# NVIDIA/flowtron

Hardware: AMD Instinct MI355X
Metric: mel-frames/sec training (2-flow, 80-mel) (higher is better)
Workload: dtype bf16; 1 GPU; BASELINE configs[1]: 2-flow LJS config.json model, per-GPU batch 32, T_max=862, L_max=157, attn-prior + CTC on, fwd+loss+bwd+clip+RAdam; global_batch=32, parallelism=dp1, mfma_operands=bf16, storage=fp32, skipped_steps=0

## Files before the change

### flowtron_amd/_lib.py

```python
from __future__ import annotations

import ctypes as C
import os

import torch

_HERE = os.path.dirname(os.path.abspath(__file__))
LIB_PATH = os.path.join(_HERE, "libflowtron_hip.so")

FT_F32, FT_BF16, FT_F16 = 0, 1, 2
GEMM_SPLITK = 1
GEMM_SPLITK_DET = 2
GEMM_C16 = 4
ACT_NONE, ACT_TANH, ACT_RELU, ACT_SIGMOID = 0, 1, 2, 3

_p, _i, _l, _f, _sz, _d = C.c_void_p, C.c_int, C.c_int64, C.c_float, C.c_size_t, C.c_double


class GemmArgs(C.Structure):
    _fields_ = [("A", _p), ("B", _p), ("C", _p), ("bias", _p),
                ("M", _i), ("N", _i), ("K", _i), ("batch", _i),
                ("sAm", _l), ("sAk", _l), ("sBk", _l), ("sBn", _l), ("ldc", _l),
                ("bsA", _l), ("bsB", _l), ("bsC", _l),
                ("alpha", _f), ("beta", _f), ("act", _i), ("mode", _i), ("flags", _i),
# ... 9 lines not shown


class GemmImgPlan(C.Structure):
    _fields_ = [(n, _i) for n in ("tile_rows", "stage_k", "gather", "atomics", "det", "splits", "chunk_w")]


class GemmImgGroupPlan(C.Structure):
    _fields_ = [(n, _i) for n in ("tile_rows", "splits", "ksteps", "atomics", "launch", "unit0", "tiles")]


GEMM_GROUP_MAX = 48


class LstmFwdRole(C.Structure):
    _fields_ = [("gx", _p), ("lens", _p), ("y", _p), ("ldy", _l), ("gates", _p), ("cell", _p), ("wimg", _p), ("state_h", _p), ("state_c", _p),
                ("B", C.c_int32), ("ldb", C.c_int32), ("t0", C.c_int32), ("t1", C.c_int32), ("gx16", C.c_int32)]


class LstmBwdRole(C.Structure):
    _fields_ = [("dy", _p), ("ldy", _l), ("lens", _p), ("gates", _p), ("cell", _p), ("dgx", _p), ("wimg", _p),
                ("dimg", _p), ("dimg_ld", _l), ("dimg_rows", _l), ("dbias", _p), ("state_da", _p), ("state_dc", _p),
                ("B", C.c_int32), ("ldb", C.c_int32), ("t0", C.c_int32), ("t1", C.c_int32), ("carry_in", C.c_int32)]


class ImgDesc(C.Structure):
    _fields_ = [("src", _p), ("ld", _l), ("rows", _l), ("cols", _l), ("dst", _p), ("kind", _i)]


class CummAttnArgs(C.Structure):
    _fields_ = [(n, _p) for n in ("text", "Q", "V", "w_key", "v", "w1", "b1", "w2", "b2", "in_lens", "ctx", "attn", "logprob",
                                  "cumm_all", "kproj_all", "work")] + [("work_bytes", _sz)] + [
        (n, _i) for n in ("T", "B", "L", "E", "A", "NF", "K1", "K2")] + [("temperature", _f), ("mode", _i), ("persist_status", _p)]


class DecodeArgs(C.Structure):
    _fields_ = [(n, _p) for n in (
        "att_w_ih", "att_w_hh", "att_b_ih", "att_b_hh", "w_query", "v", "K", "V",
# ... 60 lines not shown
    "ft_lstm_persist_workspace_bytes": ([_i, _i], _sz),
    "ft_lstm_persist_debug_prof": ([_p], _i),
    "ft_lstm_persist_bwd": ([_p, _l, _p, _p, _p, _p, _p, _p, _p, _i, _i, _i, _i, _p], _i),
    "ft_bilstm_persist_supported": ([_i, _i], _i),
    "ft_bilstm_persist_workspace_bytes": ([_i, _i], C.c_size_t),
    "ft_bilstm_persist_debug_prof": ([_p], _i),
    "ft_bilstm_persist_fwd": ([_p, _p, _p, _p, _p, _p, _l, _p, _p, _p, _p, _p, _p, _i, _i, _i, _p], _i),
    "ft_bilstm_persist_bwd": ([_p, _l, _p, _p, _p, _p, _p, _p, _p, _p, _p, _p, _p, _i, _i, _i, _p], _i),
    "ft_lstm_persist_bwd_img": ([_p, _l, _p, _p, _p, _p, _p, _p, _p, _i, _i, _i, _i, _p, _l, _l, _p, _p], _i),
    "ft_lstm_roles_ctx_bytes": ([], _sz),
    "ft_lstm_roles_wimg_bytes": ([_i], _sz),
    "ft_lstm_roles_ctx_init": ([_p, _p], _i),
    "ft_lstm_roles_debug_prof": ([_p], _i),
    "ft_lstm_roles_prepare_fwd": ([_p, _p, _i, _p], _i),
    "ft_lstm_roles_prepare_bwd": ([_p, _p, _i, _p], _i),
    "ft_lstm_roles_fwd": ([C.POINTER(LstmFwdRole), _i, _i, _i, _p, _i, _p, _i, _p], _i),
    "ft_lstm_roles_bwd": ([C.POINTER(LstmBwdRole), _i, _i, _i, _p, _i, _p, _i, _p], _i),
    "ft_lstm2_supported": ([_i, _i], _i),
    "ft_lstm2_workspace_bytes": ([_i, _i], _sz),
    "ft_lstm2_seq_fwd": ([_p] * 13 + [_i, _i, _i, _p], _i),
    "ft_lstm2_seq_bwd": ([_p] * 12 + [_i, _i, _i, _p], _i),
    "ft_lstm_bidir_supported": ([_i, _i], _i),
    "ft_lstm_bidir_seq_fwd": ([_p] * 6 + [_l] + [_p] * 6 + [_i, _i, _i, _p], _i),
    "ft_lstm_bidir_seq_bwd": ([_p, _l] + [_p] * 11 + [_i, _i, _i, _p], _i),
    "ft_cumm_attn_workspace_bytes": ([_i] * 10, _sz),
    "ft_cumm_attn_fused": ([C.POINTER(CummAttnArgs)], _i),
    "ft_cumm_attn_debug_prof": ([_p], _i),
    "ft_cumm_attn_fwd": ([C.POINTER(CummAttnArgs), _p], _i),
    "ft_cumm_attn_bwd": ([C.POINTER(CummAttnArgs)] + [_p] * 13, _i),
    "ft_attention_fwd": ([_p] * 8 + [_i, _i, _i, _i, _f, _p], _i),
# ... 72 lines not shown
    "ft_radam_step": ([_p, _p, _p, _p, _l, _p, _d, _d, _d, _d, _d, _d, _d, _i, _p, _p], _i),
    "ft_radam_step_dev": ([_p, _p, _p, _p, _l, _p, _d, _d, _d, _d, _d, _d, _i, _p, _p], _i),
    "ft_poison_if_nonzero": ([_p, _p, _p], _i),
    "ft_mixture_nll_work_floats": ([_i, _i, _i, _i], _sz),
    "ft_mixture_nll_fwd": ([_p] * 5 + [_i, _l] + [_p] * 4 + [_i] * 5 + [_p], _i),
    "ft_mixture_nll_bwd": ([_p] * 13 + [_i] * 5 + [_p], _i),
    "ft_time_pool_fwd": ([_p, _p, _p, _i, _i, _i, _p], _i),
    "ft_time_pool_bwd": ([_p, _p, _p, _i, _i, _i, _p], _i),
    "ft_softmax_rows_fwd": ([_p, _p, _i, _i, _p], _i),
    "ft_softmax_rows_bwd": ([_p, _p, _p, _i, _i, _p], _i),
    "ft_mixture_sample": ([_p] * 6 + [_i] * 5 + [_f, _p], _i),
}
MIXTURE_MAX_C = 64

OP16_TWINS = ("ft_gemm", "ft_bf16_image", "ft_bf16_image_colsum", "ft_bf16_image_colsum_acc", "ft_bf16_image_rows_acc", "ft_bf16_image_rows_act_bwd_acc", "ft_gemm_img", "ft_gemm_img_group", "ft_bf16_image_rows", "ft_bf16_image_rows_into", "ft_bf16_image_rows_act_bwd", "ft_img_gemv_rows", "ft_img_gemv_rows_bwd", "ft_lstm_seq_fwd", "ft_lstm_seq_bwd",
              "ft_lstm_persist_bwd", "ft_lstm_persist_bwd_img", "ft_lstm_roles_prepare_fwd", "ft_lstm_roles_prepare_bwd", "ft_lstm_roles_fwd", "ft_lstm_roles_bwd", "ft_lstm2_seq_fwd", "ft_lstm2_seq_bwd",
              "ft_lstm_bidir_seq_fwd", "ft_lstm_bidir_seq_bwd", "ft_bilstm_persist_fwd", "ft_bilstm_persist_bwd")
for _n in OP16_TWINS:
    SIGNATURES[_n + "_f16"] = SIGNATURES[_n]

_lib = None


def lib():
    global _lib
    if _lib is None:
        if not os.path.exists(LIB_PATH):
            raise RuntimeError(
                "libflowtron_hip.so is missing (%s). Build it with `python -m flowtron_amd.build` "
                "(hipcc --offload-arch=gfx950). There is no CPU/PyTorch fallback." % LIB_PATH)
        l = C.CDLL(LIB_PATH)
# ... 60 lines not shown
```

### flowtron_amd/csrc/lstm_roles.hip

```cpp
#include "lstm_persist_common.h"

namespace {

constexpr int CPG = 32, UPC = 32, TPC = 8;
constexpr int RMAX = 16;
constexpr int SBMAX = 32;
constexpr int RRING = 8, RDIST = 6;

constexpr int NBUF = 4;
constexpr size_t FWD_SET_DW = (size_t)8 * NBUF * (NCHUNK * 32 * RMAX / 2);
constexpr size_t BWD_SET_FL = (size_t)2 * 8 * 32 * 32 * 32 * RMAX;
constexpr size_t CTX_BYTES = 256 + 2 * FWD_SET_DW * 4 + 2 * BWD_SET_FL * 4;

struct FwdRoleP {
    const float* gx; const int* lens; float* y; long ldy; float* gates; float* cell;
    const unsigned short* wfrag;
    float* st_h; float* st_c;
    int B, LB, t0, t1;
};
struct FwdLaunchP {
    FwdRoleP role[2];
    int nroles;
    unsigned* hand;
    unsigned* census;
    int phase, reset_rows;
    int* status; long timeout_ticks; long* prof;
};

template <typename T>
__device__ __forceinline__ T* uniform_ptr(T* p) {
    const unsigned long long v = (unsigned long long)p;
    const unsigned lo = (unsigned)__builtin_amdgcn_readfirstlane((int)(unsigned)v), hi = (unsigned)__builtin_amdgcn_readfirstlane((int)(unsigned)(v >> 32));
    return (T*)(((unsigned long long)hi << 32) | lo);
}

__device__ __forceinline__ void dma16(const float* src, unsigned lds_addr) {
    unsigned keep;
    asm volatile("s_mov_b32 %0, m0\n\ts_mov_b32 m0, %2\n\ts_nop 0\n\tglobal_load_lds_dwordx4 %1, off\n\ts_mov_b32 m0, %0"
                 : "=&s"(keep) : "v"(src), "s"((unsigned)__builtin_amdgcn_readfirstlane((int)lds_addr)) : "memory");
}

__device__ __forceinline__ void preset_other(uint4* other, size_t n16, unsigned* census_other, int wg, int tid) {
    const uint4 v = {SENT, SENT, SENT, SENT};
    for (size_t i = (size_t)wg * 256 + tid; i < n16; i += (size_t)NCU * 256) other[i] = v;
    if (wg == 0 && tid < 8) census_other[tid] = 0u;
}

template <int R, bool PROF, bool GX16>
__global__ __launch_bounds__(256, 1) void lstm_roles_fwd_k(FwdLaunchP P) {
    constexpr bool SPLIT = R >= 8;
    constexpr int ERW = SPLIT ? 8 : 4;
    constexpr int EPT = R / ERW;
    constexpr int ETH = SPLIT ? 256 : 128;
    constexpr int NE = R * UPC;
    constexpr int CPL = 16 / R, NLG = 8 / CPL;
    constexpr int SBF = R == 16 ? 4 : SBMAX * 4 / R;
    constexpr int SB = GX16 ? 2 * SBF : SBF;
    constexpr int DWG = NCHUNK * 32 * R / 2;
    extern __shared__ __attribute__((aligned(16))) float smem[];
    float (*red)[4][TPC][R][20] = reinterpret_cast<float (*)[4][TPC][R][20]>(smem);
    float* gxs = smem + 2 * 4 * TPC * R * 20;
    float* outs = gxs + SBF * 4 * NE;

    const int tid = threadIdx.x, lane = tid & 63, wave = tid >> 6;
// ... 28 lines not shown
#pragma unroll
    for (int e = 0; e < EPT; ++e) {
        const int eb = b0 + er0 + ERW * e;
        ev[e] = erole && eb < B;
        len[e] = ev[e] ? p.lens[eb] : 0;
    }
    int tg = 0;
    for (int r = 0; r < R; ++r) {
        const int bb = b0 + r;
        if (bb < B) { const int l = p.lens[bb]; tg = l > tg ? l : tg; }
    }
    tg = tg < t1 ? tg : t1;
    tg = __builtin_amdgcn_readfirstlane(tg);

    const int wu = __builtin_amdgcn_readfirstlane(wave);
    auto burst = [&](int t) {
        __syncthreads();
        const int nst = (tg - t) < SB ? (tg - t) : SB;
        const unsigned dst0 = (unsigned)(size_t)(lds_void*)gxs;
        if constexpr (GX16) {
            const unsigned short* gx16 = reinterpret_cast<const unsigned short*>(p.gx);
#pragma unroll
            for (int kk = 0; kk < SB * R / 16; ++kk) {
                const int c = 4 * kk + wu, st = c / (R / 4), pi = c % (R / 4);
                const int f = pi * 512 + lane * 8, gate = f / NE, row = (f % NE) >> 5, unit = f & 31;
                if (st < nst && b0 + row < B)
                    dma16(reinterpret_cast<const float*>(gx16 + (((size_t)(t + st) * LB + b0 + row) * 4 + gate) * PH + q * UPC + unit),
                          dst0 + (unsigned)(st * 4 * NE * 2 + pi * 1024));
            }
        } else {
#pragma unroll
            for (int kk = 0; kk < SB * R / 8; ++kk) {
                const int c = 4 * kk + wu, st = c / (R / 2), pi = c % (R / 2);
                const int f = pi * 256 + lane * 4, gate = f / NE, row = (f % NE) >> 5, unit = f & 31;
                if (st < nst && b0 + row < B)
// ... 651 lines not shown
            }
        }
        if (t0 == 0) {
            int Rr = 0;
            for (int bb = 0; bb < B; ++bb) Rr += p.lens[bb] + 1;
            int Rz = (Rr + 32 + 255) & ~255;
            Rz = Rz < p.dimg_rows ? Rz : p.dimg_rows;
            for (int r = Rr + lgrp * CPG + q; r < Rz; r += gpr * CPG) {
                uint4* row = reinterpret_cast<uint4*>(p.dimg + (size_t)r * p.dimg_ld);
                for (int c = tid; c < 4 * PH / 8; c += 256) row[c] = make_uint4(0u, 0u, 0u, 0u);
            }
        }
    }
}

}

#if FT_OPFMT == 0
long* ftint_roles_prof = nullptr;
extern "C" int ft_lstm_roles_debug_prof(void* dev_buf) { ftint_roles_prof = reinterpret_cast<long*>(dev_buf); return FT_OK; }
extern "C" size_t ft_lstm_roles_ctx_bytes(void) { return CTX_BYTES; }
extern "C" size_t ft_lstm_roles_wimg_bytes(int H) { return (size_t)4 * H * H * 2; }
extern "C" int ft_lstm_roles_ctx_init(void* ctx, void* stream) {
    FT_CHECK_ARG(ctx && reinterpret_cast<uintptr_t>(ctx) % 256 == 0);
    hipStream_t st = reinterpret_cast<hipStream_t>(stream);
    FT_CHECK_HIP(hipMemsetAsync(ctx, 0, 256, st));
    FT_CHECK_HIP(hipMemsetAsync(reinterpret_cast<char*>(ctx) + 256, 0xFF, CTX_BYTES - 256, st));
    return FT_OK;
}
#else
// ... 5 lines not shown
extern "C" int FT_OPNAME(ft_lstm_roles_prepare_fwd)(const float* w_hh, void* wimg, int H, void* stream) {
    FT_CHECK_ARG(w_hh && wimg && H == PH && reinterpret_cast<uintptr_t>(wimg) % 256 == 0);
    hipLaunchKernelGGL(make_wfrag_fwd_ug, dim3(2048), dim3(256), 0, reinterpret_cast<hipStream_t>(stream), w_hh,
                       reinterpret_cast<unsigned short*>(wimg), H, WfragAux{nullptr, 0ul, 0u, nullptr});
    FT_CHECK_LAUNCH();
    return FT_OK;
}
extern "C" int FT_OPNAME(ft_lstm_roles_prepare_bwd)(const float* w_hh, void* wimg, int H, void* stream) {
    FT_CHECK_ARG(w_hh && wimg && H == PH && reinterpret_cast<uintptr_t>(wimg) % 256 == 0);
    hipLaunchKernelGGL(make_wfrag_rs, dim3(2048), dim3(256), 0, reinterpret_cast<hipStream_t>(stream), w_hh,
                       reinterpret_cast<unsigned short*>(wimg), H, WfragAux{nullptr, 0ul, 0u, nullptr});
    FT_CHECK_LAUNCH();
    return FT_OK;
}

template <typename K, typename PT>
static int roles_launch(K kern, size_t lds, const PT& P, hipStream_t st) {
    FT_CHECK_HIP(hipFuncSetAttribute(reinterpret_cast<const void*>(kern), hipFuncAttributeMaxDynamicSharedMemorySize, (int)lds));
    hipLaunchKernelGGL(kern, dim3(NCU), dim3(256), lds, st, P);
    return FT_OK;
}

extern "C" int FT_OPNAME(ft_lstm_roles_fwd)(const ft_lstm_fwd_role* roles, int n_roles, int rows_per_group, int reset_rows, void* ctx, int phase,
                                            int32_t* status, int H, void* stream) {
    FT_CHECK_ARG(roles && ctx && status && (n_roles == 1 || n_roles == 2) && reinterpret_cast<uintptr_t>(ctx) % 256 == 0 && phase >= 0);
    const int R = rows_per_group;
    FT_CHECK_ARG((R == 4 || R == 8 || R == 16) && (reset_rows == 4 || reset_rows == 8 || reset_rows == 16) && reset_rows >= 4);
    if (H != PH || !ft_lstm_persist_supported(8, H))
        return ft_fail(FT_EUNSUPPORTED, "ft_lstm_roles_fwd: needs H == 1024 and a 256-CU device (H=%d)", H);
    FwdLaunchP P{};
    bool any = false, g16 = false;
    for (int i = 0; i < n_roles; ++i) {
        const ft_lstm_fwd_role& r = roles[i];
        FT_CHECK_ARG(r.gx && r.lens && r.y && r.wimg && r.B >= 1 && r.B <= (8 / n_roles) * R && r.ldb >= r.B && r.ldy >= H);
        FT_CHECK_ARG((r.gates == nullptr) == (r.cell == nullptr) && (r.state_h == nullptr) == (r.state_c == nullptr));
        FT_CHECK_ARG(r.t0 >= 0 && r.t1 >= r.t0 && (r.t0 == 0 || r.state_h) && reinterpret_cast<uintptr_t>(r.gx) % 16 == 0);
        P.role[i] = FwdRoleP{reinterpret_cast<const float*>(r.gx), r.lens, r.y, (long)r.ldy, r.gates, r.cell, reinterpret_cast<const unsigned short*>(r.wimg),
                             r.state_h, r.state_c, r.B, r.ldb, r.t0, r.t1};
        FT_CHECK_ARG(i == 0 || (r.gx16 != 0) == g16);
        g16 = r.gx16 != 0;
        any = any || r.t1 > r.t0;
    }
    if (!any) return ft_fail(FT_EINVAL, "ft_lstm_roles_fwd: every window is empty (t1 == t0): nothing to launch");
    char* base = reinterpret_cast<char*>(ctx);
    P.nroles = n_roles;
    P.census = reinterpret_cast<unsigned*>(base);
    P.hand = reinterpret_cast<unsigned*>(base + 256);
    P.phase = phase; P.reset_rows = reset_rows;
    P.status = status; P.timeout_ticks = 100000000L / 2; P.prof = ftint_roles_prof;
    hipStream_t st = reinterpret_cast<hipStream_t>(stream);
    auto lds = [](int R_, int SB_) { return sizeof(float) * ((size_t)2 * 4 * TPC * R_ * 20 + (size_t)SB_ * 4 * R_ * UPC + (size_t)2 * 6 * R_ * UPC); };
    int rc;
    const bool pf = ftint_roles_prof != nullptr;
#define FT_ROLES_FWD(R_, SB_) \
    (g16 ? (pf ? roles_launch(lstm_roles_fwd_k<R_, true, true>, lds(R_, SB_), P, st) : roles_launch(lstm_roles_fwd_k<R_, false, true>, lds(R_, SB_), P, st)) \
         : (pf ? roles_launch(lstm_roles_fwd_k<R_, true, false>, lds(R_, SB_), P, st) : roles_launch(lstm_roles_fwd_k<R_, false, false>, lds(R_, SB_), P, st)))
    if (R == 4) rc = FT_ROLES_FWD(4, 32);
    else if (R == 8) rc = FT_ROLES_FWD(8, 16);
    else rc = FT_ROLES_FWD(16, 4);
#undef FT_ROLES_FWD
    if (rc != FT_OK) return rc;
    FT_CHECK_LAUNCH();
    return FT_OK;
}

extern "C" int FT_OPNAME(ft_lstm_roles_bwd)(const ft_lstm_bwd_role* roles, int n_roles, int rows_per_group, int reset_rows, void* ctx, int phase,
                                            int32_t* status, int H, void* stream) {
    FT_CHECK_ARG(roles && ctx && status && (n_roles == 1 || n_roles == 2) && reinterpret_cast<uintptr_t>(ctx) % 256 == 0 && phase >= 0);
    const int R = rows_per_group;
    FT_CHECK_ARG((R == 4 || R == 8 || R == 16) && (reset_rows == 4 || reset_rows == 8 || reset_rows == 16));
    if (H != PH || !ft_lstm_persist_supported(8, H))
        return ft_fail(FT_EUNSUPPORTED, "ft_lstm_roles_bwd: needs H == 1024 and a 256-CU device (H=%d)", H);
// ... 33 lines not shown
```

### flowtron_amd/ops.py

```python
from __future__ import annotations

import ctypes as C
from typing import List, Optional, Sequence

import torch

from . import _lib as L



def _c(t: torch.Tensor) -> torch.Tensor:
    return t if t.is_contiguous() else t.contiguous()


import os as _os
_BF16_IMAGES = True


def gemm_raw(A, B, Cm, M, N, K, sAm, sAk, sBk, sBn, ldc, bias=None, act=L.ACT_NONE, alpha=1.0, beta=0.0,
             batch=1, bsA=0, bsB=0, bsC=0, mode=None, splitk=False):
    L.require_cuda(A, B, Cm, bias)
    a = L.GemmArgs(L.ptr(A), L.ptr(B), L.ptr(Cm), L.ptr(bias), M, N, K, batch,
                   sAm, sAk, sBk, sBn, ldc, bsA, bsB, bsC, alpha, beta, act,
                   L.mfma_mode() if mode is None else mode, L.GEMM_SPLITK if splitk else 0,
# ... 140 lines not shown
                    "ft_bf16_image_rows_into")
            off += K
        return self

    @classmethod
    def empty_rows(cls, cols, rowmap, mode, device):
        self = cls.__new__(cls)
        self.rows, self.cols, self.fmt, self.rowmap = rowmap.cap, int(cols), mode, rowmap
        self.ld = (self.cols + 255) // 256 * 256
        self.buf = torch.empty(L.lib().ft_bf16_image_bytes(self.rows, self.cols), device=device, dtype=torch.uint8)
        self.colsum = zeroed((self.cols,), device)
        return self


_WIMG_ON = True
_WIMG = {"plan": {}, "plan_next": None, "cache": {}, "armed": False, "plans": None}


def weight_images_begin(model):
    if not _WIMG_ON:
        return
    w = _WIMG
    if w["plans"] is None:
        w["plans"] = _weakref.WeakKeyDictionary()
    w["plan"] = w["plans"].get(model, {})
    w["plan_next"], w["cache"], w["armed"] = {}, {}, bool(w["plan"])


def weight_images_end(model):
    w = _WIMG
    if w["plan_next"] is not None and w["plans"] is not None:
        w["plans"][model] = w["plan_next"]
    w["plan"], w["plan_next"], w["cache"], w["armed"] = {}, None, {}, False


import weakref as _weakref
_IMG_CACHE = {}


def shared_image(t, rows, cols, mode, rowmap=None):
    key = id(t)
    hit = _IMG_CACHE.get(key)
    want_rows = rows if rowmap is None else rowmap.cap
    if hit is not None:
        ref, ver, img = hit
        if ref() is t and ver == t._version and img.rows == want_rows and img.cols == cols and img.fmt == mode and img.rowmap is rowmap:
            return img
    img = Bf16Image(t.reshape(rows, cols), mode=mode, rowmap=rowmap)
# ... 940 lines not shown


_ROLES_CTX = {}


def roles_ctx(device):
    device = torch.device(device)
    if device.index is None:
        device = torch.device("cuda", torch.cuda.current_device())
    c = _ROLES_CTX.get(device)
    if c is None:
        c = _ROLES_CTX[device] = RolesCtx(device)
    return c


def roles_wimg(w_hh, mode, backward):
    img = torch.empty(L.lib().ft_lstm_roles_wimg_bytes(w_hh.shape[1]), device=w_hh.device, dtype=torch.uint8)
    fn = L.op16("ft_lstm_roles_prepare_bwd" if backward else "ft_lstm_roles_prepare_fwd", mode)
    w = _c(w_hh)
    L.check(fn(L.ptr(w), L.ptr(img), w.shape[1], L.stream()), "ft_lstm_roles_prepare")
    return img


def fwd_role(gx, lens, y, gates, cell, wimg, t0=0, t1=None, state=None, b0=0, nb=None):
    T, LB, H = gx.shape[0], gx.shape[1], y.shape[2]
    nb = LB - b0 if nb is None else nb
    return L.LstmFwdRole(gx.data_ptr() + gx.element_size() * 4 * H * b0, lens.data_ptr() + 4 * b0, y.data_ptr() + 4 * y.stride(1) * b0, y.stride(1),
                         gates.data_ptr() + 16 * H * b0 if gates is not None else None, cell.data_ptr() + 4 * H * b0 if cell is not None else None,
                         L.ptr(wimg), L.ptr(state[0]) if state is not None else None, L.ptr(state[1]) if state is not None else None,
                         nb, LB, t0, T if t1 is None else t1, int(gx.dtype != torch.float32))


def bwd_role(dy, lens, gates, cell, dgx, wimg, t0=0, t1=None, state=None, carry_in=False, dimg=None, b0=0, nb=None):
    T, LB, H = gates.shape[0], gates.shape[1], cell.shape[2]
    nb = LB - b0 if nb is None else nb
    return L.LstmBwdRole(dy.data_ptr() + 4 * dy.stride(1) * b0, dy.stride(1), lens.data_ptr() + 4 * b0, gates.data_ptr() + 16 * H * b0,
                         cell.data_ptr() + 4 * H * b0, dgx.data_ptr() + 16 * H * b0 if dgx is not None else None, L.ptr(wimg),
                         L.ptr(dimg.buf) if dimg is not None else None, dimg.ld if dimg is not None else 0,
                         dimg.buf.numel() // (2 * dimg.ld) if dimg is not None else 0, L.ptr(dimg.colsum) if dimg is not None else None,
# ... 335 lines not shown
            _dw_other_gradient(w_hh)
        if dW is not None and T > 1:
            rows, rm, fwd = (T - 1) * B, ctx.rowmap, not ctx.reverse
            if not images_apply(ctx.mode, 4 * H, H, rows):
                gemm_raw(dgx[1:] if fwd else dgx[:-1], y[:-1] if fwd else y[1:], dW, 4 * H, H, rows, 1, 4 * H, H, 1, H, mode=ctx.mode, splitk=True)
            elif rm is not None:
                if d_img is None:
                    d_img = Bf16Image(dgx.reshape(T * B, 4 * H), colsum=True, mode=ctx.mode, rowmap=rm)
                _compact_dw(w_hh, d_img, y_image(y, T * B, H, ctx.mode, rm), dW, 1)
            else:
                d_img, y_img = Bf16Image(dgx.reshape(T * B, 4 * H), colsum=True, mode=ctx.mode), shared_image(y, T * B, H, ctx.mode)
                weight_grad_gemm(w_hh, dW, d_img, d_img.ptr(B if fwd else 0), y_img, y_img.ptr(0 if fwd else B), dW, 4 * H, H, rows, H, beta=1.0)
        return _leave_dgates(dgx, d_img, (T, B, 4 * H), ctx.gx_dtype), dW, None, None, None, None, None


MAX_STEP_BATCH = 64


def batch_chunks(B, cap):
    return [(b0, min(cap, B - b0)) for b0 in range(0, B, cap)]


def lstm_layer(x, lens, w_ih, w_hh, b_ih, b_hh, reverse=False, mode=None, xs_extra=None, rowmap=None, fill="", gate=None):
    mode = L.mfma_mode() if mode is None else mode
    xs = [x] if xs_extra is None else [x] + list(xs_extra)
    if reverse:
        rowmap = None
    T, B = x.shape[0], x.shape[1]
    H = w_hh.shape[1]
    if lstm_pad_width(B, H, reverse, mode, x.device, T):
        w_ih_p, w_hh_p, b_p = pad_gate_blocks(w_ih, 0), pad_gate_blocks(w_hh, PERSIST_H - H), pad_gate_blocks(bias_sum(b_ih, b_hh), 0)
        out = lstm_layer(x, lens, w_ih_p, w_hh_p, b_p, torch.zeros_like(b_p), reverse, mode, xs_extra, rowmap, fill, gate)
        return out[..., :H].contiguous() if gate is None else (out[0][..., :H].contiguous(), out[1])
    gx, gates, private = _input_projection(xs, w_ih, bias_sum(b_ih, b_hh), H, reverse, mode, rowmap, fill, gate)
    if B > MAX_STEP_BATCH and not lstm_persistent(B, H, reverse, mode, gx.device):
        h = torch.cat([LSTMSeqFn.apply(gx[:, b0:b0 + nb].contiguous(), w_hh, lens[b0:b0 + nb], reverse, mode, None, False)
                       for b0, nb in batch_chunks(B, MAX_STEP_BATCH)], 1)
    else:
        h = LSTMSeqFn.apply(gx, w_hh, lens, reverse, mode, rowmap, private)
    return h if gate is None else (h, gates)


class BiLSTMSeqFn(torch.autograd.Function):

    @staticmethod
    def forward(ctx, gx_f, gx_r, w_f, w_r, lens, mode=L.FT_BF16):
        ctx.mode = mode
        gx_f, gx_r, w_f, w_r = _c(gx_f), _c(gx_r), _c(w_f), _c(w_r)
# ... 770 lines not shown
```

### include/flowtron_hip.h

```cpp
#ifndef FLOWTRON_HIP_H
#define FLOWTRON_HIP_H

#include <stddef.h>
#include <stdint.h>

#ifdef __cplusplus
extern "C" {
#endif

#define FT_ABI_VERSION 15

enum { FT_OK = 0, FT_EINVAL = -1, FT_EHIP = -2, FT_EUNSUPPORTED = -3 };
enum { FT_F32 = 0, FT_BF16 = 1, FT_F16 = 2 };
enum { FT_ACT_NONE = 0, FT_ACT_TANH = 1, FT_ACT_RELU = 2, FT_ACT_SIGMOID = 3 };
enum { FT_GEMM_SPLITK = 1, FT_GEMM_SPLITK_DET = 2, FT_GEMM_C16 = 4 };

int ft_abi_version(void);
const char* ft_last_error(void);
int ft_debug_hold_cus(int n_wg, int64_t ticks, void* stream);

typedef struct {
    const float* A; const float* B; float* C; const float* bias;
    int M, N, K, batch;
    int64_t sAm, sAk, sBk, sBn, ldc;
// ... 96 lines not shown
int ft_lstm_persist_supported(int B, int H);
size_t ft_lstm_persist_workspace_bytes(int B, int H);
int ft_lstm_persist_debug_prof(void* dev_buf);
int ft_lstm_persist_bwd(const float* dy, int64_t ldy, const float* w_hh, const int32_t* lens, const float* gates,
                        const float* cell, float* dgx, void* work, int32_t* status, int T, int B, int H, int ng, void* stream);
int ft_lstm_persist_bwd_img(const float* dy, int64_t ldy, const float* w_hh, const int32_t* lens, const float* gates,
                            const float* cell, float* dgx, void* work, int32_t* status, int T, int B, int H, int ng,
                            void* dimg, int64_t dimg_ld, int64_t dimg_rows, float* dbias, void* stream);

typedef struct {
    const void* gx; const int32_t* lens; float* y; int64_t ldy; float* gates; float* cell;
    const void* wimg;
    float* state_h; float* state_c;
    int32_t B, ldb, t0, t1;
    int32_t gx16;
} ft_lstm_fwd_role;
typedef struct {
    const float* dy; int64_t ldy; const int32_t* lens; const float* gates; const float* cell;
    float* dgx;
    const void* wimg;
    void* dimg; int64_t dimg_ld; int64_t dimg_rows; float* dbias;
    float* state_da; float* state_dc;
    int32_t B, ldb, t0, t1, carry_in;
} ft_lstm_bwd_role;
size_t ft_lstm_roles_ctx_bytes(void);
size_t ft_lstm_roles_wimg_bytes(int H);
int ft_lstm_roles_ctx_init(void* ctx, void* stream);
int ft_lstm_roles_debug_prof(void* dev_buf);
int ft_lstm_roles_prepare_fwd(const float* w_hh, void* wimg, int H, void* stream);
int ft_lstm_roles_prepare_bwd(const float* w_hh, void* wimg, int H, void* stream);
int ft_lstm_roles_fwd(const ft_lstm_fwd_role* roles, int n_roles, int rows_per_group, int reset_rows, void* ctx, int phase,
                      int32_t* status, int H, void* stream);
int ft_lstm_roles_bwd(const ft_lstm_bwd_role* roles, int n_roles, int rows_per_group, int reset_rows, void* ctx, int phase,
                      int32_t* status, int H, void* stream);

int ft_lstm2_supported(int B, int H);
size_t ft_lstm2_workspace_bytes(int B, int H);
int ft_lstm2_seq_fwd(const float* gx0, const float* w_hh0, const float* w_ih1, const float* bias1, const float* w_hh1,
                     const int32_t* lens, float* y0, float* gates0, float* cell0, float* y1, float* gates1, float* cell1,
                     void* work, int T, int B, int H, void* stream);
int ft_lstm2_seq_bwd(const float* dy1, const float* w_hh0, const float* w_ih1, const float* w_hh1, const int32_t* lens,
                     const float* gates0, const float* cell0, const float* gates1, const float* cell1,
                     float* dgx0, float* dgx1, void* work, int T, int B, int H, void* stream);

int ft_lstm_bidir_supported(int B, int H);
// ... 279 lines not shown
int ft_bf16_image_rows_f16(const float* src, int64_t ld, int64_t cap_rows, int64_t cols, void* dst, float* colsum,
                           const int32_t* rowmap, const int32_t* rows_dev, void* stream);
int ft_lstm_seq_fwd_f16(const float* gx, const float* w_hh, const int32_t* lens,
                    float* y, int64_t ldy, float* gates, float* cell, void* work,
                    int T, int B, int H, int reverse, int mode, void* stream);
int ft_lstm_seq_bwd_f16(const float* dy, int64_t ldy, const float* w_hh, const int32_t* lens,
                    const float* gates, const float* cell, float* dgx, void* work,
                    int T, int B, int H, int reverse, int mode, void* stream);
int ft_lstm_persist_bwd_f16(const float* dy, int64_t ldy, const float* w_hh, const int32_t* lens, const float* gates,
                        const float* cell, float* dgx, void* work, int32_t* status, int T, int B, int H, int ng, void* stream);
int ft_lstm_persist_bwd_img_f16(const float* dy, int64_t ldy, const float* w_hh, const int32_t* lens, const float* gates,
                            const float* cell, float* dgx, void* work, int32_t* status, int T, int B, int H, int ng,
                            void* dimg, int64_t dimg_ld, int64_t dimg_rows, float* dbias, void* stream);
int ft_lstm_roles_prepare_fwd_f16(const float* w_hh, void* wimg, int H, void* stream);
int ft_lstm_roles_prepare_bwd_f16(const float* w_hh, void* wimg, int H, void* stream);
int ft_lstm_roles_fwd_f16(const ft_lstm_fwd_role* roles, int n_roles, int rows_per_group, int reset_rows, void* ctx, int phase,
                          int32_t* status, int H, void* stream);
int ft_lstm_roles_bwd_f16(const ft_lstm_bwd_role* roles, int n_roles, int rows_per_group, int reset_rows, void* ctx, int phase,
                          int32_t* status, int H, void* stream);
int ft_lstm2_seq_fwd_f16(const float* gx0, const float* w_hh0, const float* w_ih1, const float* bias1, const float* w_hh1,
                     const int32_t* lens, float* y0, float* gates0, float* cell0, float* y1, float* gates1, float* cell1,
                     void* work, int T, int B, int H, void* stream);
int ft_lstm2_seq_bwd_f16(const float* dy1, const float* w_hh0, const float* w_ih1, const float* w_hh1, const int32_t* lens,
                     const float* gates0, const float* cell0, const float* gates1, const float* cell1,
                     float* dgx0, float* dgx1, void* work, int T, int B, int H, void* stream);
int ft_lstm_bidir_seq_fwd_f16(const float* gx_f, const float* gx_r, const float* w_hh_f, const float* w_hh_r,
                          const int32_t* lens, float* y, int64_t ldy, float* gates_f, float* gates_r,
                          float* cell_f, float* cell_r, void* work_f, void* work_r, int T, int B, int H, void* stream);
int ft_lstm_bidir_seq_bwd_f16(const float* dy, int64_t ldy, const float* w_hh_f, const float* w_hh_r, const int32_t* lens,
                          const float* gates_f, const float* gates_r, const float* cell_f, const float* cell_r,
// ... 13 lines not shown
```

Before: 743,100 mel-frames/s.

## Fuse LSTM input projection into persistent roles kernel and batch weight-fragment prep

```diff
diff --git a/flowtron_amd/_lib.py b/flowtron_amd/_lib.py
--- a/flowtron_amd/_lib.py
+++ b/flowtron_amd/_lib.py
@@ -47,13 +47,18 @@
 
 class LstmFwdRole(C.Structure):
     _fields_ = [("gx", _p), ("lens", _p), ("y", _p), ("ldy", _l), ("gates", _p), ("cell", _p), ("wimg", _p), ("state_h", _p), ("state_c", _p),
-                ("B", C.c_int32), ("ldb", C.c_int32), ("t0", C.c_int32), ("t1", C.c_int32), ("gx16", C.c_int32)]
+                ("B", C.c_int32), ("ldb", C.c_int32), ("t0", C.c_int32), ("t1", C.c_int32), ("gx16", C.c_int32),
+                ("x_img", _p), ("wih_img", _p), ("x_bias", _p), ("x_ld", _l), ("wih_ld", _l), ("x_rows", _l), ("xproj_k", C.c_int32)]
 
 
 class LstmBwdRole(C.Structure):
     _fields_ = [("dy", _p), ("ldy", _l), ("lens", _p), ("gates", _p), ("cell", _p), ("dgx", _p), ("wimg", _p),
                 ("dimg", _p), ("dimg_ld", _l), ("dimg_rows", _l), ("dbias", _p), ("state_da", _p), ("state_dc", _p),
                 ("B", C.c_int32), ("ldb", C.c_int32), ("t0", C.c_int32), ("t1", C.c_int32), ("carry_in", C.c_int32)]
+
+
+class WfragDesc(C.Structure):
+    _fields_ = [("w_hh", _p), ("fwd_img", _p), ("bwd_img", _p)]
 
 
 class ImgDesc(C.Structure):
@@ -144,6 +149,7 @@
     "ft_lstm_roles_debug_prof": ([_p], _i),
     "ft_lstm_roles_prepare_fwd": ([_p, _p, _i, _p], _i),
     "ft_lstm_roles_prepare_bwd": ([_p, _p, _i, _p], _i),
+    "ft_lstm_roles_prepare_table": ([C.POINTER(WfragDesc), _i, _i, _p], _i),
     "ft_lstm_roles_fwd": ([C.POINTER(LstmFwdRole), _i, _i, _i, _p, _i, _p, _i, _p], _i),
     "ft_lstm_roles_bwd": ([C.POINTER(LstmBwdRole), _i, _i, _i, _p, _i, _p, _i, _p], _i),
     "ft_lstm2_supported": ([_i, _i], _i),
@@ -246,7 +252,7 @@
 MIXTURE_MAX_C = 64
 
 OP16_TWINS = ("ft_gemm", "ft_bf16_image", "ft_bf16_image_colsum", "ft_bf16_image_colsum_acc", "ft_bf16_image_rows_acc", "ft_bf16_image_rows_act_bwd_acc", "ft_gemm_img", "ft_gemm_img_group", "ft_bf16_image_rows", "ft_bf16_image_rows_into", "ft_bf16_image_rows_act_bwd", "ft_img_gemv_rows", "ft_img_gemv_rows_bwd", "ft_lstm_seq_fwd", "ft_lstm_seq_bwd",
-              "ft_lstm_persist_bwd", "ft_lstm_persist_bwd_img", "ft_lstm_roles_prepare_fwd", "ft_lstm_roles_prepare_bwd", "ft_lstm_roles_fwd", "ft_lstm_roles_bwd", "ft_lstm2_seq_fwd", "ft_lstm2_seq_bwd",
+              "ft_lstm_persist_bwd", "ft_lstm_persist_bwd_img", "ft_lstm_roles_prepare_fwd", "ft_lstm_roles_prepare_bwd", "ft_lstm_roles_prepare_table", "ft_lstm_roles_fwd", "ft_lstm_roles_bwd", "ft_lstm2_seq_fwd", "ft_lstm2_seq_bwd",
               "ft_lstm_bidir_seq_fwd", "ft_lstm_bidir_seq_bwd", "ft_bilstm_persist_fwd", "ft_bilstm_persist_bwd")
 for _n in OP16_TWINS:
     SIGNATURES[_n + "_f16"] = SIGNATURES[_n]
diff --git a/flowtron_amd/csrc/lstm_roles.hip b/flowtron_amd/csrc/lstm_roles.hip
--- a/flowtron_amd/csrc/lstm_roles.hip
+++ b/flowtron_amd/csrc/lstm_roles.hip
@@ -17,6 +17,8 @@
     const unsigned short* wfrag;
     float* st_h; float* st_c;
     int B, LB, t0, t1;
+    const unsigned short* ximg; const unsigned short* wih; const float* xbias;
+    long xld, wld; int xrows, K;
 };
 struct FwdLaunchP {
     FwdRoleP role[2];
@@ -27,6 +29,21 @@
     int* status; long timeout_ticks; long* prof;
 };
 
+__device__ __forceinline__ void mfma16_v_first(f32x4& acc, const bf16x8& a, const bf16x8& b) {
+#if FT_OPFMT == 1
+    asm volatile("s_nop 1\n\tv_mfma_f32_16x16x32_f16 %0, %1, %2, 0" : "=&v"(acc) : "v"(a), "v"(b));
+#else
+    asm volatile("s_nop 1\n\tv_mfma_f32_16x16x32_bf16 %0, %1, %2, 0" : "=&v"(acc) : "v"(a), "v"(b));
+#endif
+}
+__device__ __forceinline__ void mfma16_v(f32x4& acc, const bf16x8& a, const bf16x8& b) {
+#if FT_OPFMT == 1
+    asm volatile("s_nop 1\n\tv_mfma_f32_16x16x32_f16 %0, %1, %2, %0" : "+v"(acc) : "v"(a), "v"(b));
+#else
+    asm volatile("s_nop 1\n\tv_mfma_f32_16x16x32_bf16 %0, %1, %2, %0" : "+v"(acc) : "v"(a), "v"(b));
+#endif
+}
+
 template <typename T>
 __device__ __forceinline__ T* uniform_ptr(T* p) {
     const unsigned long long v = (unsigned long long)p;
@@ -46,8 +63,9 @@
     if (wg == 0 && tid < 8) census_other[tid] = 0u;
 }
 
-template <int R, bool PROF, bool GX16>
+template <int R, bool PROF, bool GX16, bool XP = false>
 __global__ __launch_bounds__(256, 1) void lstm_roles_fwd_k(FwdLaunchP P) {
+    static_assert(!XP || (GX16 && R <= 8), "computed bursts: the 16-bit burst layout, 4 or 8 rows per group");
     constexpr bool SPLIT = R >= 8;
     constexpr int ERW = SPLIT ? 8 : 4;
     constexpr int EPT = R / ERW;
@@ -106,11 +124,73 @@
     tg = __builtin_amdgcn_readfirstlane(tg);
 
     const int wu = __builtin_amdgcn_readfirstlane(wave);
+    int xbase = 0, xlen = 0;
+    bool xok = false;
+    if constexpr (XP) {
+        const int xb = b0 + (li & (R - 1));
+        xok = xb < B;
+        if (xok) {
+            for (int i = 0; i < xb; ++i) { const int l = p.lens[i]; xbase += (l < 0 ? 0 : l) + 1; }
+            xlen = p.lens[xb];
+            xlen = xlen < 0 ? 0 : xlen;
+        }
+    }
     auto burst = [&](int t) {
         __syncthreads();
         const int nst = (tg - t) < SB ? (tg - t) : SB;
         const unsigned dst0 = (unsigned)(size_t)(lds_void*)gxs;
-        if constexpr (GX16) {
+        if constexpr (XP) {
+            constexpr int SPT = 16 / R;
+            const int K = p.K, nk = (K + 31) >> 5;
+            const bf16x8 zero8 = {0, 0, 0, 0, 0, 0, 0, 0};
+            bf16x8 xf[4][4];
+#pragma unroll
+            for (int i = 0; i < 4; ++i) {
+                const int st = (4 * i + wu) * SPT + (li / R);
+                int tt = t + st;
+                tt = tt < xlen ? tt : xlen;
+                int ri = xbase + tt;
+                ri = ri < p.xrows ? ri : p.xrows - 1;
+                const unsigned short* xr = p.ximg + (size_t)ri * p.xld + kg * 8;
+#pragma unroll
+                for (int ks = 0; ks < 4; ++ks)
+                    xf[i][ks] = (xok && (4 * i + wu) * SPT < nst && ks * 32 + kg * 8 < K) ? *reinterpret_cast<const bf16x8*>(xr + ks * 32) : zero8;
+            }
+            auto wload = [&](int jt, bf16x8 (&wf)[4], f32x4& bias) {
+                const int col = (jt >> 1) * PH + q * UPC + (jt & 1) * 16;
+                const unsigned short* wr = p.wih + (size_t)(col + li) * p.wld + kg * 8;
+#pragma unroll
+                for (int ks = 0; ks < 4; ++ks) wf[ks] = (ks * 32 + kg * 8 < K) ? *reinterpret_cast<const bf16x8*>(wr + ks * 32) : zero8;
+                bias = *reinterpret_cast<const f32x4*>(p.xbias + col + kg * 4);
+            };
+            bf16x8 wf[2][4];
+            f32x4 bs[2];
+            wload(0, wf[0], bs[0]);
+            unsigned short* const gxs16 = reinterpret_cast<unsigned short*>(gxs);
+#pragma unroll
+            for (int jt = 0; jt < 8; ++jt) {
+                if (jt + 1 < 8) wload(jt + 1, wf[(jt + 1) & 1], bs[(jt + 1) & 1]);
+                f32x4 acc[4];
+#pragma unroll
+                for (int i = 0; i < 4; ++i) mfma16_v_first(acc[i], wf[jt & 1][0], xf[i][0]);
+#pragma unroll
+                for (int ks = 1; ks < 4; ++ks) {
+                    if (ks >= nk) break;
+#pragma unroll
+                    for (int i = 0; i < 4; ++i) mfma16_v(acc[i], wf[jt & 1][ks], xf[i][ks]);
+                }
+                asm volatile("s_nop 7\n\ts_nop 3" : "+v"(acc[0]), "+v"(acc[1]), "+v"(acc[2]), "+v"(acc[3]));
+                const f32x4 b4 = bs[jt & 1];
+#pragma unroll
+                for (int i = 0; i < 4; ++i) {
+                    const int st = (4 * i + wu) * SPT + (li / R);
+                    uint2 pk;
+                    pk.x = pack_op16x2(acc[i][0] + b4[0], acc[i][1] + b4[1]);
+                    pk.y = pack_op16x2(acc[i][2] + b4[2], acc[i][3] + b4[3]);
+                    *reinterpret_cast<uint2*>(gxs16 + ((st * 4 + (jt >> 1)) * R + (li & (R - 1))) * UPC + (jt & 1) * 16 + kg * 4) = pk;
+                }
+            }
+        } else if constexpr (GX16) {
             const unsigned short* gx16 = reinterpret_cast<const unsigned short*>(p.gx);
 #pragma unroll
             for (int kk = 0; kk < SB * R / 16; ++kk) {
@@ -792,6 +872,43 @@
     }
 }
 
+constexpr int WFRAG_TABLE_MAX = 16;
+struct WfragTable {
+    const float* w[WFRAG_TABLE_MAX]; unsigned short* fwd[WFRAG_TABLE_MAX]; unsigned short* bwd[WFRAG_TABLE_MAX];
+};
+__global__ __launch_bounds__(256) void make_wfrag_table_k(WfragTable tab) {
+    constexpr int TS = 128 + 8;
+    __shared__ __attribute__((aligned(16))) unsigned short tile[128 * TS];
+    const int tid = threadIdx.x, wi = blockIdx.x >> 8, q = (blockIdx.x >> 3) & 31, cc = blockIdx.x & 7;
+    const float* __restrict__ w = tab.w[wi];
+    unsigned short* const fwd = tab.fwd[wi];
+    unsigned short* const bwd = tab.bwd[wi];
+#pragma unroll 4
+    for (int pass = 0; pass < 16; ++pass) {
+        const int row = pass * 8 + (tid >> 5), c4 = (tid & 31) * 4;
+        const float4 v = *reinterpret_cast<const float4*>(w + ((size_t)(row >> 5) * PH + q * 32 + (row & 31)) * PH + cc * 128 + c4);
+        *reinterpret_cast<uint2*>(&tile[row * TS + c4]) = make_uint2((unsigned)f2op16(v.x) | ((unsigned)f2op16(v.y) << 16),
+                                                                     (unsigned)f2op16(v.z) | ((unsigned)f2op16(v.w) << 16));
+    }
+    __syncthreads();
+#pragma unroll 2
+    for (int it = 0; it < 8; ++it) {
+        const int p = it * 256 + tid, lane = p & 63, a = (p >> 6) & 3, b = p >> 8;
+        const int li = lane & 15, kg = lane >> 4;
+        if (fwd) {
+            const uint4 v = *reinterpret_cast<const uint4*>(&tile[((li & 3) * 32 + b * 4 + (li >> 2)) * TS + a * 32 + kg * 8]);
+            *reinterpret_cast<uint4*>(fwd + ((size_t)((q * 8 + b) * NCHUNK + cc * 4 + a) * 64 + lane) * 8) = v;
+        }
+        if (bwd) {
+            unsigned s[8];
+#pragma unroll
+            for (int e = 0; e < 8; ++e) s[e] = tile[(a * 32 + kg * 8 + e) * TS + b * 16 + li];
+            *reinterpret_cast<uint4*>(bwd + ((size_t)((q * (PH / 16) + cc * 8 + b) * 4 + a) * 64 + lane) * 8) =
+                make_uint4(s[0] | (s[1] << 16), s[2] | (s[3] << 16), s[4] | (s[5] << 16), s[6] | (s[7] << 16));
+        }
+    }
+}
+
 }
 
 #if FT_OPFMT == 0
@@ -827,6 +944,20 @@
     return FT_OK;
 }
 
+extern "C" int FT_OPNAME(ft_lstm_roles_prepare_table)(const ft_wfrag_desc* descs, int n, int H, void* stream) {
+    FT_CHECK_ARG(descs && n >= 1 && n <= WFRAG_TABLE_MAX && H == PH);
+    WfragTable t{};
+    for (int i = 0; i < n; ++i) {
+        const ft_wfrag_desc& d = descs[i];
+        FT_CHECK_ARG(d.w_hh && (d.fwd_img || d.bwd_img) && reinterpret_cast<uintptr_t>(d.w_hh) % 16 == 0 &&
+                     reinterpret_cast<uintptr_t>(d.fwd_img) % 256 == 0 && reinterpret_cast<uintptr_t>(d.bwd_img) % 256 == 0);
+        t.w[i] = d.w_hh; t.fwd[i] = reinterpret_cast<unsigned short*>(d.fwd_img); t.bwd[i] = reinterpret_cast<unsigned short*>(d.bwd_img);
+    }
+    hipLaunchKernelGGL(make_wfrag_table_k, dim3(n * 256), dim3(256), 0, reinterpret_cast<hipStream_t>(stream), t);
+    FT_CHECK_LAUNCH();
+    return FT_OK;
+}
+
 template <typename K, typename PT>
 static int roles_launch(K kern, size_t lds, const PT& P, hipStream_t st) {
     FT_CHECK_HIP(hipFuncSetAttribute(reinterpret_cast<const void*>(kern), hipFuncAttributeMaxDynamicSharedMemorySize, (int)lds));
@@ -842,16 +973,26 @@
     if (H != PH || !ft_lstm_persist_supported(8, H))
         return ft_fail(FT_EUNSUPPORTED, "ft_lstm_roles_fwd: needs H == 1024 and a 256-CU device (H=%d)", H);
     FwdLaunchP P{};
-    bool any = false, g16 = false;
+    bool any = false, g16 = false, xp = false;
     for (int i = 0; i < n_roles; ++i) {
         const ft_lstm_fwd_role& r = roles[i];
-        FT_CHECK_ARG(r.gx && r.lens && r.y && r.wimg && r.B >= 1 && r.B <= (8 / n_roles) * R && r.ldb >= r.B && r.ldy >= H);
+        FT_CHECK_ARG((r.xproj_k != 0 || r.gx) && r.lens && r.y && r.wimg && r.B >= 1 && r.B <= (8 / n_roles) * R && r.ldb >= r.B && r.ldy >= H);
         FT_CHECK_ARG((r.gates == nullptr) == (r.cell == nullptr) && (r.state_h == nullptr) == (r.state_c == nullptr));
         FT_CHECK_ARG(r.t0 >= 0 && r.t1 >= r.t0 && (r.t0 == 0 || r.state_h) && reinterpret_cast<uintptr_t>(r.gx) % 16 == 0);
         P.role[i] = FwdRoleP{reinterpret_cast<const float*>(r.gx), r.lens, r.y, (long)r.ldy, r.gates, r.cell, reinterpret_cast<const unsigned short*>(r.wimg),
                              r.state_h, r.state_c, r.B, r.ldb, r.t0, r.t1};
-        FT_CHECK_ARG(i == 0 || (r.gx16 != 0) == g16);
+        if (r.xproj_k != 0) {
+            FT_CHECK_ARG(R <= 8 && r.xproj_k >= 8 && r.xproj_k <= 128 && r.xproj_k % 8 == 0 && r.x_img && r.wih_img && r.x_bias);
+            FT_CHECK_ARG(reinterpret_cast<uintptr_t>(r.x_img) % 16 == 0 && reinterpret_cast<uintptr_t>(r.wih_img) % 16 == 0 &&
+                         reinterpret_cast<uintptr_t>(r.x_bias) % 16 == 0);
+            FT_CHECK_ARG(r.x_ld >= r.xproj_k && r.x_ld % 8 == 0 && r.wih_ld >= r.xproj_k && r.wih_ld % 8 == 0 && r.x_rows >= 1 && r.x_rows < (1ll << 31));
+            FwdRoleP& fp = P.role[i];
+            fp.ximg = reinterpret_cast<const unsigned short*>(r.x_img); fp.wih = reinterpret_cast<const unsigned short*>(r.wih_img);
+            fp.xbias = r.x_bias; fp.xld = (long)r.x_ld; fp.wld = (long)r.wih_ld; fp.xrows = (int)r.x_rows; fp.K = r.xproj_k;
+        }
+        FT_CHECK_ARG(i == 0 || ((r.gx16 != 0) == g16 && (r.xproj_k != 0) == xp));
         g16 = r.gx16 != 0;
+        xp = r.xproj_k != 0;
         any = any || r.t1 > r.t0;
     }
     if (!any) return ft_fail(FT_EINVAL, "ft_lstm_roles_fwd: every window is empty (t1 == t0): nothing to launch");
@@ -868,7 +1009,9 @@
 #define FT_ROLES_FWD(R_, SB_) \
     (g16 ? (pf ? roles_launch(lstm_roles_fwd_k<R_, true, true>, lds(R_, SB_), P, st) : roles_launch(lstm_roles_fwd_k<R_, false, true>, lds(R_, SB_), P, st)) \
          : (pf ? roles_launch(lstm_roles_fwd_k<R_, true, false>, lds(R_, SB_), P, st) : roles_launch(lstm_roles_fwd_k<R_, false, false>, lds(R_, SB_), P, st)))
-    if (R == 4) rc = FT_ROLES_FWD(4, 32);
+    if (xp && R == 4) rc = pf ? roles_launch(lstm_roles_fwd_k<4, true, true, true>, lds(4, 32), P, st) : roles_launch(lstm_roles_fwd_k<4, false, true, true>, lds(4, 32), P, st);
+    else if (xp) rc = pf ? roles_launch(lstm_roles_fwd_k<8, true, true, true>, lds(8, 16), P, st) : roles_launch(lstm_roles_fwd_k<8, false, true, true>, lds(8, 16), P, st);
+    else if (R == 4) rc = FT_ROLES_FWD(4, 32);
     else if (R == 8) rc = FT_ROLES_FWD(8, 16);
     else rc = FT_ROLES_FWD(16, 4);
 #undef FT_ROLES_FWD
diff --git a/flowtron_amd/ops.py b/flowtron_amd/ops.py
--- a/flowtron_amd/ops.py
+++ b/flowtron_amd/ops.py
@@ -178,7 +178,8 @@
 
 
 _WIMG_ON = True
-_WIMG = {"plan": {}, "plan_next": None, "cache": {}, "armed": False, "plans": None}
+_WIMG = {"plan": {}, "plan_next": None, "cache": {}, "armed": False, "plans": None,
+         "wf_plan": {}, "wf_plan_next": None, "wf_cache": {}, "wf_armed": False, "wf_plans": None, "wf_last": None, "wf_grad": False}
 
 
 def weight_images_begin(model):
@@ -186,9 +187,12 @@
         return
     w = _WIMG
     if w["plans"] is None:
-        w["plans"] = _weakref.WeakKeyDictionary()
+        w["plans"], w["wf_plans"] = _weakref.WeakKeyDictionary(), _weakref.WeakKeyDictionary()
     w["plan"] = w["plans"].get(model, {})
     w["plan_next"], w["cache"], w["armed"] = {}, {}, bool(w["plan"])
+    w["wf_plan"] = w["wf_plans"].get(model, {})
+    w["wf_plan_next"], w["wf_cache"], w["wf_armed"], w["wf_last"] = {}, {}, bool(w["wf_plan"]), None
+    w["wf_grad"] = torch.is_grad_enabled()
 
 
 def weight_images_end(model):
@@ -196,6 +200,10 @@
     if w["plan_next"] is not None and w["plans"] is not None:
         w["plans"][model] = w["plan_next"]
     w["plan"], w["plan_next"], w["cache"], w["armed"] = {}, None, {}, False
+    if w["wf_plan_next"] is not None and w["wf_plans"] is not None:
+        w["wf_plans"][model] = w["wf_last"] = w["wf_plan_next"]
+    w["wf_cache"] = {k: v for k, v in w["wf_cache"].items() if k[1]}
+    w["wf_plan"], w["wf_plan_next"], w["wf_armed"] = {}, None, False
 
 
 import weakref as _weakref
@@ -1166,7 +1174,48 @@
     return c
 
 
+WFRAG_TABLE_MAX = 16
+
+
+def _wfrag_planned(w_hh, mode, backward):
+    w = _WIMG
+    key = (w_hh.data_ptr(), tuple(w_hh.shape), mode)
+    if backward:
+        e = w["wf_last"].get(key) if w["wf_last"] is not None else None
+        if e is not None:
+            e[1] = True
+    elif w["wf_plan_next"] is not None and isinstance(w_hh, torch.nn.Parameter) and w_hh.shape[1] == PERSIST_H:
+        prev = w["wf_plan"].get(key)
+        w["wf_plan_next"][key] = [w_hh, bool(prev is not None and prev[1])]
+    if w["wf_armed"] and not backward:
+        w["wf_armed"] = False
+        nbytes = L.lib().ft_lstm_roles_wimg_bytes(PERSIST_H)
+        plan = [(k, t, bw) for k, (t, bw) in w["wf_plan"].items() if t.is_cuda and t.device == w_hh.device and t.dtype == torch.float32
+                and t.is_contiguous() and t.data_ptr() == k[0] and tuple(t.shape) == k[1]]
+        for fmt in sorted({k[2] for k, _, _ in plan}):
+            items = [p for p in plan if p[0][2] == fmt]
+            for lo in range(0, len(items), WFRAG_TABLE_MAX):
+                part = items[lo:lo + WFRAG_TABLE_MAX]
+                descs = (L.WfragDesc * len(part))()
+                for i, (k, t, bw) in enumerate(part):
+                    f_img = torch.empty(nbytes, device=t.device, dtype=torch.uint8)
+                    b_img = torch.empty(nbytes, device=t.device, dtype=torch.uint8) if bw and w["wf_grad"] else None
+                    descs[i] = L.WfragDesc(t.data_ptr(), L.ptr(f_img), L.ptr(b_img))
+                    w["wf_cache"][(k, False)] = (f_img, t, t._version)
+                    if b_img is not None:
+                        w["wf_cache"][(k, True)] = (b_img, t, t._version)
+                L.check(L.op16("ft_lstm_roles_prepare_table", fmt)(descs, len(part), PERSIST_H, L.stream()), "ft_lstm_roles_prepare_table")
+    hit = w["wf_cache"].pop((key, bool(backward)), None)
+    if hit is not None and hit[2] == w_hh._version:
+        return hit[0]
+    return None
+
+
 def roles_wimg(w_hh, mode, backward):
+    if _WIMG_ON:
+        img = _wfrag_planned(w_hh, mode, backward)
+        if img is not None:
+            return img
     img = torch.empty(L.lib().ft_lstm_roles_wimg_bytes(w_hh.shape[1]), device=w_hh.device, dtype=torch.uint8)
     fn = L.op16("ft_lstm_roles_prepare_bwd" if backward else "ft_lstm_roles_prepare_fwd", mode)
     w = _c(w_hh)
@@ -1174,7 +1223,16 @@
     return img
 
 
-def fwd_role(gx, lens, y, gates, cell, wimg, t0=0, t1=None, state=None, b0=0, nb=None):
+def fwd_role(gx, lens, y, gates, cell, wimg, t0=0, t1=None, state=None, b0=0, nb=None, xproj=None):
+    if xproj is not None:
+        x_img, w_img, bias = xproj
+        assert gx is None and b0 == 0 and x_img.fmt == w_img.fmt and x_img.cols == w_img.cols and bias.dtype == torch.float32
+        T, LB = y.shape[0], y.shape[1]
+        nb = LB if nb is None else nb
+        return L.LstmFwdRole(None, lens.data_ptr(), y.data_ptr(), y.stride(1), L.ptr(gates), L.ptr(cell), L.ptr(wimg),
+                             L.ptr(state[0]) if state is not None else None, L.ptr(state[1]) if state is not None else None,
+                             nb, LB, t0, T if t1 is None else t1, 0,
+                             x_img.ptr(), w_img.ptr(), L.ptr(bias), x_img.ld, w_img.ld, x_img.rows, x_img.cols)
     T, LB, H = gx.shape[0], gx.shape[1], y.shape[2]
     nb = LB - b0 if nb is None else nb
     return L.LstmFwdRole(gx.data_ptr() + gx.element_size() * 4 * H * b0, lens.data_ptr() + 4 * b0, y.data_ptr() + 4 * y.stride(1) * b0, y.stride(1),
@@ -1540,6 +1598,62 @@
         return _leave_dgates(dgx, d_img, (T, B, 4 * H), ctx.gx_dtype), dW, None, None, None, None, None
 
 
+_XPROJ = True
+XPROJ_MAX_K = 128
+
+
+def xproj_ok(mode, rowmap, T, B, H, reverse, xs, N, gate, device):
+    if not (_XPROJ and gate is None and len(xs) == 1 and xs[0].shape[-1] <= XPROJ_MAX_K and xs[0].shape[-1] % 8 == 0):
+        return False
+    if not gx16_ok(mode, rowmap, T, B, H, reverse, xs, N, device):
+        return False
+    plan = roles_plan(B, False)
+    return len(plan) == 1 and plan[0][2] <= 8
+
+
+class _NodeCtx:
+
+    def __init__(self, saved_tensors, needs_input_grad, **attrs):
+        self.saved_tensors, self.needs_input_grad = saved_tensors, needs_input_grad
+        self.__dict__.update(attrs)
+
+
+class LSTMProjSeqFn(torch.autograd.Function):
+
+    @staticmethod
+    def forward(ctx, x, w_ih, bias, w_hh, lens, mode, rowmap, fill):
+        x, w_ih, bias, w_hh = _c(x), _c(w_ih), _c(bias), _c(w_hh)
+        L.require_cuda(x, w_ih, bias, w_hh, lens)
+        if bias.data_ptr() % 16:
+            bias = bias.clone()
+        T, B, K = x.shape
+        H = w_hh.shape[1]
+        w_img = Bf16Image.of_weight(w_ih, mode)
+        x_img = shared_image(x, T * B, K, mode, rowmap)
+        y, gates, cell = (torch.empty(T, B, n, device=x.device, dtype=torch.float32) for n in (H, 4 * H, H))
+        wimg = roles_wimg(w_hh, mode, False)
+        (_, _, R), = roles_plan(B, False)
+        roles_launch([fwd_role(None, lens, y, gates, cell, wimg, xproj=(x_img, w_img, bias))], R, mode, x.device)
+        ctx.imgs = (w_img, [x_img])
+        ctx.save_for_backward(x, w_ih, w_hh, lens, y, gates, cell)
+        ctx.mode, ctx.rowmap, ctx.fill = mode, rowmap, fill
+        return y
+
+    @staticmethod
+    def backward(ctx, dy):
+        x, w_ih, w_hh, lens, y, gates, cell = ctx.saved_tensors
+        need = ctx.needs_input_grad
+        rec = _NodeCtx((w_hh, lens, y, gates, cell), (False, need[3]), reverse=False, mode=ctx.mode, rowmap=ctx.rowmap, gx_private=True,
+                       gx_dtype=op16_dtype(ctx.mode))
+        dgx, dW_hh = LSTMSeqFn.backward(rec, dy)[:2]
+        lin = _NodeCtx((w_ih, None, x), (need[1], need[2], False, False, False, False, need[0]), imgs=ctx.imgs, img_kind="images",
+                       lazy_img_mode=None, lazy_src=None, has_bias=True, act=L.ACT_NONE, rowmap=ctx.rowmap, fill=ctx.fill, cat=False,
+                       mode=ctx.mode, mode_dx=ctx.mode, mode_dw=ctx.mode)
+        g = LinearFn.backward(lin, dgx)
+        ctx.imgs = None
+        return g[6], g[0], g[1], dW_hh, None, None, None, None
+
+
 MAX_STEP_BATCH = 64
 
 
@@ -1558,6 +1672,8 @@
         w_ih_p, w_hh_p, b_p = pad_gate_blocks(w_ih, 0), pad_gate_blocks(w_hh, PERSIST_H - H), pad_gate_blocks(bias_sum(b_ih, b_hh), 0)
         out = lstm_layer(x, lens, w_ih_p, w_hh_p, b_p, torch.zeros_like(b_p), reverse, mode, xs_extra, rowmap, fill, gate)
         return out[..., :H].contiguous() if gate is None else (out[0][..., :H].contiguous(), out[1])
+    if xproj_ok(mode, rowmap, T, B, H, reverse, xs, w_ih.shape[0], gate, x.device):
+        return LSTMProjSeqFn.apply(x, w_ih, bias_sum(b_ih, b_hh), w_hh, lens, mode, rowmap, fill)
     gx, gates, private = _input_projection(xs, w_ih, bias_sum(b_ih, b_hh), H, reverse, mode, rowmap, fill, gate)
     if B > MAX_STEP_BATCH and not lstm_persistent(B, H, reverse, mode, gx.device):
         h = torch.cat([LSTMSeqFn.apply(gx[:, b0:b0 + nb].contiguous(), w_hh, lens[b0:b0 + nb], reverse, mode, None, False)
diff --git a/include/flowtron_hip.h b/include/flowtron_hip.h
--- a/include/flowtron_hip.h
+++ b/include/flowtron_hip.h
@@ -134,6 +134,9 @@
     float* state_h; float* state_c;
     int32_t B, ldb, t0, t1;
     int32_t gx16;
+    const void* x_img; const void* wih_img; const float* x_bias;
+    int64_t x_ld, wih_ld, x_rows;
+    int32_t xproj_k;
 } ft_lstm_fwd_role;
 typedef struct {
     const float* dy; int64_t ldy; const int32_t* lens; const float* gates; const float* cell;
@@ -149,6 +152,8 @@
 int ft_lstm_roles_debug_prof(void* dev_buf);
 int ft_lstm_roles_prepare_fwd(const float* w_hh, void* wimg, int H, void* stream);
 int ft_lstm_roles_prepare_bwd(const float* w_hh, void* wimg, int H, void* stream);
+typedef struct { const float* w_hh; void* fwd_img; void* bwd_img; } ft_wfrag_desc;
+int ft_lstm_roles_prepare_table(const ft_wfrag_desc* descs, int n, int H, void* stream);
 int ft_lstm_roles_fwd(const ft_lstm_fwd_role* roles, int n_roles, int rows_per_group, int reset_rows, void* ctx, int phase,
                       int32_t* status, int H, void* stream);
 int ft_lstm_roles_bwd(const ft_lstm_bwd_role* roles, int n_roles, int rows_per_group, int reset_rows, void* ctx, int phase,
@@ -458,6 +463,7 @@
                             void* dimg, int64_t dimg_ld, int64_t dimg_rows, float* dbias, void* stream);
 int ft_lstm_roles_prepare_fwd_f16(const float* w_hh, void* wimg, int H, void* stream);
 int ft_lstm_roles_prepare_bwd_f16(const float* w_hh, void* wimg, int H, void* stream);
+int ft_lstm_roles_prepare_table_f16(const ft_wfrag_desc* descs, int n, int H, void* stream);
 int ft_lstm_roles_fwd_f16(const ft_lstm_fwd_role* roles, int n_roles, int rows_per_group, int reset_rows, void* ctx, int phase,
                           int32_t* status, int H, void* stream);
 int ft_lstm_roles_bwd_f16(const ft_lstm_bwd_role* roles, int n_roles, int rows_per_group, int reset_rows, void* ctx, int phase,
```

New measurement: 752,500 mel-frames/s (median of 6 runs). +1.3%, better.
